# li199603/easy_gaussian_splatting

Hardware: AMD Instinct MI355X
Metric: train iters/sec + forward render fps, 1M Gaussians @ 1080p (higher is better)
Workload: dtype f32

## Files before the change

### easy_gaussian_splatting_amd/csrc/gs_blend.hip

```cpp
#include <algorithm>

#include "gs_common.h"
#include "gs_math.h"

namespace gs {

#ifdef GS_BWD_CHECK
struct BwdCheck {
    float* fwd_T;
    int32_t* fwd_cnt;
    float2* unit_out;
    int2* unit_hdr;
};
static BwdCheck g_bwd_check = {nullptr, nullptr, nullptr, nullptr};
#define GS_IF_CHECK(...) __VA_ARGS__
#else
#define GS_IF_CHECK(...)
#endif

constexpr int kUnit = GS_UNIT;
constexpr int kChunk = 8;
constexpr int kUnitLog = 128;
constexpr int kWalkUnits = GS_WALK_UNITS, kWalkStorage = GS_WALK_STORAGE, kWalkRows = GS_WALK_ROWS,
              kWalkFlags = GS_WALK_FLAGS, kWalkSkip = GS_WALK_SKIP;
constexpr int kScanThreads = 256, kScanPerThread = 32, kScanChunk = kScanThreads * kScanPerThread;

struct BlendFwdArgs {
    const int32_t* tile_order;
    int C, W, H, tw, tiles;
    const float4* rec;
    const float* bg;
    const int32_t *isect_offsets, *flatten_ids, *slots;
    float *out_colors, *out_alphas;
    float4* ckpt;
    int2* qlist;
    int32_t* qcnt;
    uint8_t* qmask;
// ... 153 lines not shown
        if (CKPT) {
            const int4 rc = a.trec[2 * (size_t)t], ru = a.trec[2 * (size_t)t + 1];
            cnt[0] = __builtin_amdgcn_readfirstlane(rc.x); cnt[1] = __builtin_amdgcn_readfirstlane(rc.y);
            cnt[2] = __builtin_amdgcn_readfirstlane(rc.z); cnt[3] = __builtin_amdgcn_readfirstlane(rc.w);
            const int ru4[4] = {ru.x, ru.y, ru.z, ru.w};
#pragma unroll
            for (int k = 0; k < 4; ++k) {
                room[k] = -cnt[k] & (kUnit - 1);
                if (lane == 0 && cnt[k] > 0) uring[4 * k + (((cnt[k] - 1) / kUnit) & 3)] = ru4[k];
            }
        }
    }
    const float qxlo[2] = {(float)x0 + 0.5f, (float)x0 + 8.5f}, qxhi[2] = {(float)x0 + 7.5f, (float)x0 + 15.5f};
    const float qylo[2] = {(float)y0 + 0.5f, (float)y0 + 8.5f}, qyhi[2] = {(float)y0 + 7.5f, (float)y0 + 15.5f};

    auto publish = [&]() {
        if (log_n == 0) return;
        int base = 0;
        if (lane == 0) base = atomicAdd(a.walk + kWalkUnits, log_n);
        base = __builtin_amdgcn_readfirstlane(base);
        __builtin_amdgcn_wave_barrier();
        for (int j = lane; j < log_n; j += 64) {
            const int2 e = ulog[j];
            if (base + j < a.cap_units) a.unit_desc[base + j] = make_int4(4 * t + (e.y & 3), e.y >> 2, e.x, 0);
        }
        __builtin_amdgcn_wave_barrier();
        log_n = 0;
    };

    for (int b = 0; b < nb; ++b) {
        bool qa[4];
#pragma unroll
        for (int k = 0; k < 4; ++k) qa[k] = __builtin_amdgcn_ballot_w64(px_live(T[k])) != 0ull;
        if (!(qa[0] || qa[1] || qa[2] || qa[3])) break;
        if (CKPT && log_n > kUnitLog - 8) publish();
        const int first = lo + b * GS_BUCKET;
        const int m = min(GS_BUCKET, hi - first);
        bool hx[2] = {false, false}, hy[2] = {false, false};
        int my_gid = 0, my_slot = 0;
        if (lane < m) {
            my_gid = a.flatten_ids[first + lane];
            if (CKPT) my_slot = a.slots[first + lane];
            const float4* r = a.rec + 3 * (size_t)my_gid;
            const float4 q0 = r[0], q1 = r[1], q2 = r[2];
            srec[lane * 3] = q0; srec[lane * 3 + 1] = q1; srec[lane * 3 + 2] = q2;
            const float ex = q1.z, ey = q1.w;
#pragma unroll
// ... 32 lines not shown
                    const bool ok = px_live(T[k]) && sigma >= 0.f && alpha >= kAlphaMin;
                    const float am = ok ? alpha : 0.f;
                    if (CKPT) {
                        if (__builtin_amdgcn_ballot_w64(ok) != 0ull) {
                            if (__builtin_expect(room[k] == 0, 0)) {
                                const int pos = cnt[k] + (int)__popcll(cq[k]);
                                if (pool_left == 0) {
                                    int base = 0;
                                    if (lane == 0) base = atomicAdd(range_ctr, kChunk);
                                    base = __builtin_amdgcn_readfirstlane(base);
                                    if (base + kChunk > range_len) {
                                        if (lane == 0) {
                                            atomicOr(a.walk + kWalkFlags, GS_FLAG_UNITS);
                                            if (ROUND != 1 && a.flags) atomicOr(a.flags, (unsigned long long)GS_FLAG_UNITS);
                                        }
                                        base = 0;
                                    }
                                    pool_next = range0 + base; pool_left = kChunk;
                                }
                                const int su = pool_next++;
                                --pool_left;
                                a.ckpt[(size_t)su * 64 + lane] = make_float4(px_live(T[k]) ? T[k] : -1.f, cr[k], cg[k], cb[k]);
                                if constexpr (NC == 4) ckpt_ext[(size_t)su * 64 + lane] = ca[k];
                                if (lane == 0) ulog[log_n] = make_int2(su, (pos / kUnit) * 4 + k);
                                ++log_n;
                                if (lane == 0) uring[4 * k + ((pos / kUnit) & 3)] = su;
                                room[k] = kUnit;
                            }
                            --room[k];
                            cq[k] |= 1ull << j;
                        }
                    }
                    GS_IF_CHECK(const float T_before = T[k];)
                    if constexpr (NC == 4) blend_masked4(am, r, g, bl, q2.w, T[k], cr[k], cg[k], cb[k], ca[k]);
                    else blend_masked(am, r, g, bl, T[k], cr[k], cg[k], cb[k]);
                    GS_IF_CHECK(taken[k] += T[k] < T_before ? 1 : 0;)
                }
            }
        }
        if (CKPT) {
            int mybits = 0;
#pragma unroll
            for (int k = 0; k < 4; ++k) {
                const int n_new = (int)__popcll(cq[k]);
                if ((cq[k] >> lane) & 1) {
                    const int p = cnt[k] + (int)__popcll(cq[k] & lt_mask);
                    const int su = uring[4 * k + ((p / kUnit) & 3)];
// ... 149 lines not shown
    const int32_t tot = row_counts32(a.qmask, i0, n, w);
    int32_t block_tot;
    const int32_t run = block_excl_scan_add<int32_t>(tot, scratch, &block_tot) + a.walk[GS_WALK_WORDS + blockIdx.x];
    int32_t first16 = 0;
#pragma unroll
    for (int j = 0; j < 4; ++j) first16 += (int32_t)((w[j] * 0x01010101u) >> 24);
    if (i0 <= n) a.row_base[i0 >> 4] = run;
    if (i0 + 16 <= n) a.row_base[(i0 >> 4) + 1] = run + first16;
}

struct BlendBwdArgs {
    int C, W, H, tw, tiles;
    const float4* rec;
    const int32_t* walk;
    const int2* qlist;
    const int32_t* qcnt;
    const int4* unit_desc;
    const float4* ckpt;
    const uint8_t* qmask;
    const int32_t* row_base;
    int cap_units;
    const int32_t* cls_hdr;
    const int4* cls_desc;
    int cls_cap;
    const float *out_colors, *out_alphas, *v_colors, *v_alphas;
    float4* rows;
    const int64_t* guard;
    GS_IF_CHECK(BwdCheck chk;)
};

constexpr int kBwdWaves = 4;
constexpr int kPipeLanes = 8;
constexpr int kPerLane = kUnit / kPipeLanes;
static_assert(kPerLane == 4, "bwd_wave is instantiated for 1 .. 4 entries per lane");
constexpr int kUnitsPerWave = 64 / kPipeLanes;
constexpr int kUnitPixels = 64;
constexpr int kBwdSteps = kUnitPixels + kPipeLanes - 1;

__device__ __forceinline__ float dpp_row_shr1(float v) {
    return __builtin_bit_cast(float, __builtin_amdgcn_update_dpp(__builtin_bit_cast(int, v), __builtin_bit_cast(int, v), 0x111, 0xf, 0xf, false));
}


#ifdef GS_BWD_ACC64
typedef double acc_t;
#define GS_ACC_FMA(a, b, c) ((double)(a) * (double)(b) + (c))
#else
typedef float acc_t;
#define GS_ACC_FMA(a, b, c) fmaf((a), (b), (c))
#endif
struct EntryState {
    float mx, my, hA, Bc, hC, op, colr, colg, colb, At, Bt, Ct;
    acc_t s_mx, s_my, s_ax, s_ay, s_A, s_B, s_C, s_vs, s_r, s_g, s_b;
    bool has;
    float col3; acc_t s_3;
};

template <int NC>
__device__ __forceinline__ void bwd_pair(EntryState& e, const float4 d0, const float v3, const float2 d1, float& T, float& P) {
    const float dx = e.mx - d1.x, dy = e.my - d1.y;
// ... 6 lines not shown
    const float Tn = fmaf(-alpha, T, T);
    const bool stop = ok && Tn <= kTMin;
    const bool contrib = ok && !stop;
    float cv = e.colr * d0.x + e.colg * d0.y + e.colb * d0.z;
    if constexpr (NC == 4) cv = fmaf(e.col3, v3, cv);
    const float wm = contrib ? w : 0.f;
    const float Pn = fmaf(wm, cv, P);
    const float ra = fast_rcp(1.f - alpha);
    const float v_alpha = fmaf(T, cv, ra * (d0.w + Pn));
    e.s_r = GS_ACC_FMA(wm, d0.x, e.s_r); e.s_g = GS_ACC_FMA(wm, d0.y, e.s_g); e.s_b = GS_ACC_FMA(wm, d0.z, e.s_b);
    if constexpr (NC == 4) e.s_3 = GS_ACC_FMA(wm, v3, e.s_3);
    const float vs = (contrib && ov <= kAlphaMax) ? -ov * v_alpha : 0.f;
    const float hx = vs * dx, hy = vs * dy;
    e.s_A = GS_ACC_FMA(hx, dx, e.s_A); e.s_B = GS_ACC_FMA(hx, dy, e.s_B); e.s_C = GS_ACC_FMA(hy, dy, e.s_C);
    const float gx = fmaf(e.At, hx, e.Bt * hy), gy = fmaf(e.Bt, hx, e.Ct * hy);
    e.s_mx += (acc_t)gx; e.s_my += (acc_t)gy; e.s_ax += (acc_t)fabsf(gx); e.s_ay += (acc_t)fabsf(gy);
    e.s_vs += (acc_t)vs;
    T = contrib ? Tn : (stop ? -1.f : T);
    P = Pn;
}

template <int E, int NC>
__device__ __forceinline__ void bwd_wave(const BlendBwdArgs& a, const int4 ud, const bool valid, const int unit, float4* sd0, float* sd1,
                                         float2* sck, const int r, const float* __restrict__ ckpt_ext) {
    const int tq = ud.x, su = ud.z;
    const bool first_unit = ud.y == 0;
    const int t = tq >> 2, q = tq & 3;
    const int cam = t / a.tiles, tt = t - cam * a.tiles;
    const int tyi = tt / a.tw, txi = tt - tyi * a.tw;
    const int qx0 = txi * GS_TILE + 8 * (q & 1), qy0 = tyi * GS_TILE + 8 * (q >> 1);
    const float fx0 = (float)qx0 + 0.5f, fy0 = (float)qy0 + 0.5f;
    const float4* ckp = a.ckpt + (size_t)su * 64;

    const int n_sub = valid ? a.qcnt[tq] : 0;
    int2 gs[E];
    {
        const int2* qp2 = a.qlist + (size_t)su * kUnit + E * r;
        if constexpr (E == 4) {
            const int4* qp = reinterpret_cast<const int4*>(qp2);
            const int4 g0 = qp[0], g1 = qp[1];
            gs[0] = make_int2(g0.x, g0.y); gs[1] = make_int2(g0.z, g0.w); gs[2] = make_int2(g1.x, g1.y); gs[3] = make_int2(g1.z, g1.w);
        } else if constexpr (E == 2) {
            const int4 g0 = *reinterpret_cast<const int4*>(qp2);
            gs[0] = make_int2(g0.x, g0.y); gs[1] = make_int2(g0.z, g0.w);
        } else {
#pragma unroll
            for (int i = 0; i < E; ++i) gs[i] = qp2[i];
// ... 8 lines not shown
    for (int i = 0; i < kPix; ++i) {
        const int p = r + kPipeLanes * i;
        const int px = min(qx0 + (p & 7), a.W - 1), py = min(qy0 + (p >> 3), a.H - 1);
        const size_t o = ((size_t)cam * a.H + py) * a.W + px;
        l_vr[i] = a.v_colors[NC * o];
        l_vg[i] = NC > 1 ? a.v_colors[NC * o + 1] : 0.f;
        l_vb[i] = NC > 2 ? a.v_colors[NC * o + 2] : 0.f;
        l_oa[i] = a.out_alphas[o];
        l_cr[i] = a.out_colors[NC * o];
        l_cg[i] = NC > 1 ? a.out_colors[NC * o + 1] : 0.f;
        l_cb[i] = NC > 2 ? a.out_colors[NC * o + 2] : 0.f;
        l_va[i] = vap[o];
        l_ck[i] = ckp[p];
        if constexpr (NC == 4) { l_v3[i] = a.v_colors[NC * o + 3]; l_c3[i] = a.out_colors[NC * o + 3]; l_k3[i] = ckpt_ext[(size_t)su * 64 + p]; }
    }
    const int n_in = min(kPipeLanes * E, n_sub - ud.y * kUnit);
    float4 rq[E][3];
#pragma unroll
    for (int i = 0; i < E; ++i) {
        const bool has = E * r + i < n_in;
        const float4* rp = a.rec + 3 * (size_t)(has ? gs[i].x : 0);
        rq[i][0] = rp[0]; rq[i][1] = rp[1]; rq[i][2] = rp[2];
    }
#pragma unroll
    for (int i = 0; i < kPix; ++i) {
        const int p = r + kPipeLanes * i;
        const bool inside = valid && (qx0 + (p & 7)) < a.W && (qy0 + (p >> 3)) < a.H;
        const float vr = l_vr[i], vg = l_vg[i], vb = l_vb[i];
        const float Tf = 1.f - l_oa[i];
        const float va = a.v_alphas ? l_va[i] : 0.f;
        float Ev = Tf * va - (l_cr[i] * vr + l_cg[i] * vg + l_cb[i] * vb);
        const float4 ck = first_unit ? make_float4(1.f, 0.f, 0.f, 0.f) : l_ck[i];
        float Pk = ck.y * vr + ck.z * vg + ck.w * vb;
        if constexpr (NC == 4) {
            const float v3 = l_v3[i];
            Ev = Tf * va - fmaf(l_c3[i], v3, l_cr[i] * vr + l_cg[i] * vg + l_cb[i] * vb);
            Pk = fmaf(first_unit ? 0.f : l_k3[i], v3, Pk);
            sd1[p] = inside ? v3 : 0.f;
        }
        sd0[p] = inside ? make_float4(vr, vg, vb, Ev) : make_float4(0.f, 0.f, 0.f, 0.f);
        sck[p] = inside ? make_float2(ck.x, Pk) : make_float2(-1.f, 0.f);
    }

    EntryState e[E];
    int slot[E];
#pragma unroll
    for (int i = 0; i < E; ++i) {
        const int en = E * r + i;
        e[i].has = en < n_in;
        slot[i] = e[i].has ? gs[i].y : 0;
        const float4 z4 = make_float4(0.f, 0.f, 0.f, 0.f);
        const float4 q0 = e[i].has ? rq[i][0] : z4, q1 = e[i].has ? rq[i][1] : z4, q2 = e[i].has ? rq[i][2] : z4;
        e[i].mx = q0.x; e[i].my = q0.y; e[i].hA = q0.z; e[i].Bc = q0.w; e[i].hC = q1.x; e[i].op = q1.y;
        e[i].colr = q2.x; e[i].colg = q2.y; e[i].colb = q2.z;
        e[i].col3 = q2.w; e[i].s_3 = (acc_t)0;
        e[i].At = 2.f * kLn2 * q0.z; e[i].Bt = kLn2 * q0.w; e[i].Ct = 2.f * kLn2 * q1.x;
        e[i].s_mx = e[i].s_my = e[i].s_ax = e[i].s_ay = e[i].s_A = e[i].s_B = e[i].s_C = e[i].s_vs = (acc_t)0;
        e[i].s_r = e[i].s_g = e[i].s_b = (acc_t)0;
    }
    __builtin_amdgcn_wave_barrier();

    float T_out = -1.f, P_out = 0.f;
    GS_IF_CHECK(float D_out = -1.f, C_out = 0.f; if (valid && r == 0 && a.chk.unit_hdr) a.chk.unit_hdr[unit] = make_int2(tq, ud.y);)
    for (int s = 0; s < kBwdSteps; ++s) {
        float T = dpp_row_shr1(T_out), P = dpp_row_shr1(P_out);
        const int p = s - r;
        const bool act = (unsigned)p < (unsigned)kUnitPixels;
        const int pc = min(max(p, 0), kUnitPixels - 1);
        const float4 d0 = sd0[pc];
        const float v3 = NC == 4 ? sd1[pc] : 0.f;
        const float2 ck = sck[pc];
        const float2 d1 = make_float2(fx0 + (float)(pc & 7), fy0 + (float)(pc >> 3));
        if (r == 0) { T = ck.x; P = ck.y; }
        T = act ? T : -1.f;
        GS_IF_CHECK(float D = dpp_row_shr1(D_out), Cn = dpp_row_shr1(C_out); if (r == 0) { D = ck.x; Cn = 0.f; } if (!act) { D = -1.f; Cn = 0.f; })
#pragma unroll
        for (int i = 0; i < E; ++i) {
            GS_IF_CHECK(const float T_before = T;)
            bwd_pair<NC>(e[i], d0, v3, d1, T, P);
            GS_IF_CHECK(if (T > 0.f && T < T_before) { D = T; Cn += 1.f; })
        }
        GS_IF_CHECK(D_out = D; C_out = Cn;
                    if (valid && act && r == kPipeLanes - 1 && a.chk.unit_out) a.chk.unit_out[(size_t)unit * 64 + p] = make_float2(D, Cn);)
        T_out = T; P_out = P;
    }

    int row[E];
#pragma unroll
    for (int i = 0; i < E; ++i) {
        int m;
        row[i] = rows_before(a.row_base, a.qmask, slot[i], &m);
        row[i] += __popc((unsigned)m & ((1u << q) - 1u));
    }
#pragma unroll
    for (int i = 0; i < E; ++i) {
        if (e[i].has) {
            float4* rp = a.rows + (GS_ROW_FLOATS / 4) * (size_t)row[i];
            const float v_op = e[i].op > 0.f ? (float)(-e[i].s_vs / (acc_t)e[i].op) : 0.f;
            rp[0] = make_float4((float)e[i].s_mx, (float)e[i].s_my, (float)e[i].s_ax, (float)e[i].s_ay);
            rp[1] = make_float4((float)((acc_t)0.5f * e[i].s_A), (float)e[i].s_B, (float)((acc_t)0.5f * e[i].s_C), v_op);
            rp[2] = make_float4((float)e[i].s_r, (float)e[i].s_g, (float)e[i].s_b, NC == 4 ? (float)e[i].s_3 : 0.f);
        }
    }
}

constexpr int kClsHdrInts = 16, kClsThreads = 1024;
__global__ __launch_bounds__(64) void unit_classes_clear_kernel(int32_t* __restrict__ hdr) {
    if (threadIdx.x < kClsHdrInts) hdr[threadIdx.x] = 0;
}
__global__ __launch_bounds__(kClsThreads) void unit_classes_kernel(const int32_t* __restrict__ walk, const int4* __restrict__ unit_desc,
                                                                   const int32_t* __restrict__ qcnt, int cap_units, int cls_cap,
                                                                   int32_t* __restrict__ hdr, int4* __restrict__ cls, const int64_t* __restrict__ guard) {
    __shared__ int s_cnt[kClsThreads / 64][4], s_base[kClsThreads / 64][4];
    if (guard_tripped(guard)) return;
    const int n_units = min(walk[kWalkUnits], cap_units);
    if ((int)blockIdx.x * kClsThreads >= n_units) return;
    const int u = (int)blockIdx.x * kClsThreads + (int)threadIdx.x, wave = threadIdx.x >> 6, lane = threadIdx.x & 63;
    int c = 0;
    int4 ud = make_int4(0, 0, 0, 0);
    if (u < n_units) {
        ud = unit_desc[u];
        const int n_in = min(kUnit, qcnt[ud.x] - ud.y * kUnit);
        c = min(max((n_in + kPipeLanes - 1) / kPipeLanes, 1), 4);
        ud.w = u;
    }
    unsigned long long m[4];
#pragma unroll
    for (int k = 0; k < 4; ++k) m[k] = __ballot(c == k + 1);
    if (lane < 4) s_cnt[wave][lane] = (int)__popcll(lane == 0 ? m[0] : (lane == 1 ? m[1] : (lane == 2 ? m[2] : m[3])));
    __syncthreads();
    if (threadIdx.x < 4) {
        int tot = 0;
        for (int w = 0; w < kClsThreads / 64; ++w) { s_base[w][threadIdx.x] = tot; tot += s_cnt[w][threadIdx.x]; }
        const int base = tot ? atomicAdd(hdr + 1 + threadIdx.x, tot) : 0;
        for (int w = 0; w < kClsThreads / 64; ++w) s_base[w][threadIdx.x] += base;
    }
    __syncthreads();
    if (c) {
        const unsigned long long mine = c == 1 ? m[0] : (c == 2 ? m[1] : (c == 3 ? m[2] : m[3]));
        const int i = s_base[wave][c - 1] + (int)__popcll(mine & ((1ull << lane) - 1ull));
        if (i < (c == 4 ? cap_units : cls_cap)) cls[(c == 4 ? 0 : cap_units + (3 - c) * cls_cap) + i] = ud;
    }
}

template <int NC>
__device__ __forceinline__ void blend_bwd_body(const BlendBwdArgs& a, const float* __restrict__ ckpt_ext) {
    __shared__ float4 sd0_all[kBwdWaves][kUnitsPerWave][64];
    __shared__ float2 sck_all[kBwdWaves][kUnitsPerWave][64];
    const int wave = threadIdx.x >> 6, lane = threadIdx.x & 63;
    const int pipe = lane / kPipeLanes, r = lane & (kPipeLanes - 1);
    if (guard_tripped(a.guard)) return;
    constexpr int kPerBlock = kBwdWaves * kUnitsPerWave;
    int cls = 4, blk = (int)blockIdx.x, n_units, first = 0;
    if (a.cls_hdr == nullptr) {
        n_units = min(a.walk[kWalkUnits], a.cap_units);
    } else {
        const int b4 = (a.cap_units + kPerBlock - 1) / kPerBlock, bt = (a.cls_cap + kPerBlock - 1) / kPerBlock;
        if (blk >= b4) {
            const int k = (blk - b4) / bt;
            cls = 3 - k; blk -= b4 + k * bt; first = a.cap_units + k * a.cls_cap;
        }
        n_units = min(a.cls_hdr[cls], cls == 4 ? a.cap_units : a.cls_cap);
    }
    const int in_class = (blk * kBwdWaves + wave) * kUnitsPerWave + pipe;
    if ((blk * kBwdWaves + wave) * kUnitsPerWave >= n_units) return;
    GS_CLOCK_PROBE_SCOPE(2);
    const bool valid = in_class < n_units;
    float4* sd0 = sd0_all[wave][pipe];
    float2* sck = sck_all[wave][pipe];
    float* sd1 = nullptr;
    if constexpr (NC == 4) {
        __shared__ float sd1_all[kBwdWaves][kUnitsPerWave][64];
        sd1 = sd1_all[wave][pipe];
    }

    int4 ud = make_int4(0, 0, 0, 0);
    if (valid) ud = a.cls_hdr ? a.cls_desc[first + in_class] : a.unit_desc[in_class];
    const int unit = a.cls_hdr ? ud.w : in_class;
    if (cls == 4) bwd_wave<4, NC>(a, ud, valid, unit, sd0, sd1, sck, r, ckpt_ext);
    else if (cls == 3) bwd_wave<3, NC>(a, ud, valid, unit, sd0, sd1, sck, r, ckpt_ext);
    else if (cls == 2) bwd_wave<2, NC>(a, ud, valid, unit, sd0, sd1, sck, r, ckpt_ext);
    else bwd_wave<1, NC>(a, ud, valid, unit, sd0, sd1, sck, r, ckpt_ext);
}

__global__ __launch_bounds__(kBwdWaves * 64) void blend_bwd_kernel(const BlendBwdArgs a) {
    blend_bwd_body<3>(a, nullptr);
}
template <int NC>
__global__ __launch_bounds__(kBwdWaves * 64) void chan_bwd_kernel(const BlendBwdArgs a, const float* ckpt_ext) {
    blend_bwd_body<NC>(a, ckpt_ext);
}

}

using namespace gs;

#ifdef GS_BWD_CHECK
extern "C" int gs_debug_bwd_check_set(float* fwd_T, int32_t* fwd_cnt, float* unit_out, int32_t* unit_hdr) {
    g_bwd_check.fwd_T = fwd_T; g_bwd_check.fwd_cnt = fwd_cnt;
    g_bwd_check.unit_out = reinterpret_cast<float2*>(unit_out); g_bwd_check.unit_hdr = reinterpret_cast<int2*>(unit_hdr);
    return GS_OK;
}
#endif

#ifdef GS_CLOCK_PROBE
extern "C" int gs_debug_clock_probe(int64_t* out4, int reset) {
    unsigned long long h[4] = {0, 0, 0, 0};
    if (out4) { GS_HIP_CHECK(hipMemcpyFromSymbol(h, HIP_SYMBOL(gs_clk_acc), sizeof(h))); for (int i = 0; i < 4; ++i) out4[i] = (int64_t)h[i]; }
    if (reset) { unsigned long long z[4] = {0, 0, 0, 0}; GS_HIP_CHECK(hipMemcpyToSymbol(HIP_SYMBOL(gs_clk_acc), z, sizeof(z))); }
    return GS_OK;
}
#endif

extern "C" size_t gs_walk_state_ints(int64_t n_isects) {
    if (n_isects < 0) return 0;
    return (size_t)GS_WALK_WORDS + (size_t)(n_isects / kScanChunk + 1);
}

template <int NC>
static int blend_fwd_launch(void* stream, int C, int width, int height, const float* rec,
                            const float* backgrounds, const int32_t* isect_offsets, const int32_t* tile_order,
                            const int32_t* flatten_ids, const int32_t* slots, int64_t n_isects, float* render_colors,
                            float* render_alphas, float* ckpt, int32_t* qlist, int32_t* qcnt, uint8_t* qmask,
// ... 110 lines not shown
                            const int32_t* qlist, const int32_t* qcnt, const int32_t* unit_desc, int64_t cap_units,
                            const float* ckpt, const uint8_t* qmask, const int32_t* row_base, const int32_t* walk_state,
                            const float* render_colors, const float* render_alphas, const float* v_render_colors,
                            const float* v_render_alphas, float* rows, int32_t* unit_classes, const float* ckpt_ext) {
    GS_REQUIRE(C >= 1 && width > 0 && height > 0 && cap_units >= 0 && cap_units < (1ll << 26), "C>=1, positive image size, 0 <= cap_units < 2^26");
    if (cap_units == 0) return GS_OK;
    GS_REQUIRE(rec && qlist && qcnt && unit_desc && ckpt && qmask && row_base && walk_state, "null list pointer");
    GS_REQUIRE(render_colors && render_alphas && v_render_colors && rows, "null image pointer");
    GS_REQUIRE(NC != 4 || ckpt_ext, "channels = 4: ckpt_ext (gs_blend_fwd_ch's fourth-channel checkpoints) is required");
    BlendBwdArgs a;
    a.C = C; a.W = width; a.H = height;
    a.tw = (width + GS_TILE - 1) / GS_TILE;
    a.tiles = a.tw * ((height + GS_TILE - 1) / GS_TILE);
    a.rec = reinterpret_cast<const float4*>(rec);
    a.qlist = reinterpret_cast<const int2*>(qlist); a.qcnt = qcnt; a.walk = walk_state;
    a.unit_desc = reinterpret_cast<const int4*>(unit_desc); a.cap_units = (int)cap_units;
    a.ckpt = reinterpret_cast<const float4*>(ckpt); a.qmask = qmask; a.row_base = row_base;
    a.out_colors = render_colors;
    a.out_alphas = render_alphas; a.v_colors = v_render_colors; a.v_alphas = v_render_alphas;
    a.rows = reinterpret_cast<float4*>(rows);
    a.guard = current_guard().info;
    GS_IF_CHECK(a.chk = g_bwd_check;)
    unsigned grid = (unsigned)((cap_units + kUnitsPerWave * kBwdWaves - 1) / (kUnitsPerWave * kBwdWaves));
    a.cls_hdr = nullptr; a.cls_desc = nullptr; a.cls_cap = 0;
    if (unit_classes) {
        GS_REQUIRE(((uintptr_t)unit_classes & 15) == 0, "unit_classes must be 16-byte aligned");
        a.cls_hdr = unit_classes; a.cls_desc = reinterpret_cast<const int4*>(unit_classes + kClsHdrInts);
        a.cls_cap = (int)cls_region(C, width, height);
        hipLaunchKernelGGL(unit_classes_clear_kernel, dim3(1), dim3(64), 0, (hipStream_t)stream, unit_classes);
        hipLaunchKernelGGL(unit_classes_kernel, dim3((unsigned)((cap_units + kClsThreads - 1) / kClsThreads)), dim3(kClsThreads), 0, (hipStream_t)stream,
                           walk_state, a.unit_desc, qcnt, (int)cap_units, a.cls_cap, unit_classes, reinterpret_cast<int4*>(unit_classes + kClsHdrInts),
                           a.guard);
        GS_LAUNCH_CHECK("unit_classes_kernel");
        grid += 3u * (unsigned)(a.cls_cap / (kUnitsPerWave * kBwdWaves));
    }
    if constexpr (NC == 3) hipLaunchKernelGGL(blend_bwd_kernel, dim3(grid), dim3(kBwdWaves * 64), 0, (hipStream_t)stream, a);
    else hipLaunchKernelGGL((chan_bwd_kernel<NC>), dim3(grid), dim3(kBwdWaves * 64), 0, (hipStream_t)stream, a, ckpt_ext);
    GS_LAUNCH_CHECK("blend_bwd_kernel");
    return GS_OK;
}

extern "C" int gs_blend_bwd(void* stream, int C, int width, int height, const float* rec,
                            const int32_t* qlist, const int32_t* qcnt, const int32_t* unit_desc, int64_t cap_units,
                            const float* ckpt, const uint8_t* qmask, const int32_t* row_base, const int32_t* walk_state,
                            const float* render_colors, const float* render_alphas, const float* v_render_colors,
                            const float* v_render_alphas, float* rows, int32_t* unit_classes) {
    return blend_bwd_launch<3>(stream, C, width, height, rec, qlist, qcnt, unit_desc, cap_units, ckpt, qmask, row_base, walk_state,
                               render_colors, render_alphas, v_render_colors, v_render_alphas, rows, unit_classes, nullptr);
}

extern "C" int gs_blend_bwd_ch(void* stream, int C, int width, int height, int channels, const float* rec,
                               const int32_t* qlist, const int32_t* qcnt, const int32_t* unit_desc, int64_t cap_units,
                               const float* ckpt, const uint8_t* qmask, const int32_t* row_base, const int32_t* walk_state,
                               const float* render_colors, const float* render_alphas, const float* v_render_colors,
                               const float* v_render_alphas, float* rows, int32_t* unit_classes, const float* ckpt_ext) {
    GS_REQUIRE(channels >= 1 && channels <= 4, "channels must be 1, 2, 3 or 4");
#define GS_BWD_CH(NC) blend_bwd_launch<NC>(stream, C, width, height, rec, qlist, qcnt, unit_desc, cap_units, ckpt, qmask, row_base, \
// ... 11 lines not shown
```

### easy_gaussian_splatting_amd/rendering.py

```python
from __future__ import annotations

import ctypes as _ct
import math
import os
import threading
import time
import weakref
from typing import Dict, Optional, Tuple

import torch
from torch import Tensor

from . import _native as nat
from . import workspace as WS

_TILE = nat.GS_TILE
_BWD_CLASSES = os.environ.get("GS_BWD_CLASSES", "1") != "0"


def _ptr(t: Optional[Tensor]) -> Optional[int]:
    return None if t is None else t.data_ptr()


def _stream(device: torch.device) -> int:
# ... 397 lines not shown
    coarse_cap, shift, flags = lay.key[5:8]
    if flags & WS.F_TWO_LEVEL:
        check(L.gs_bins_lists(st, C, N, tw, th, shift, bbox, P(WS.BIN), lay.extent(WS.BIN), P(WS.COARSE_KEYS), coarse_cap, P(WS.CUM_TILES),
                              P(WS.ISECT_OFFSETS), P(WS.ISECT_IDS), P(WS.FLATTEN_IDS), P(WS.SLOTS), P(WS.INFO)), "gs_bins_lists")
    else:
        check(L.gs_bin_emit_sort(st, C, N, tw, th, bbox, depths, P(WS.BIN), lay.extent(WS.BIN), P(WS.ISECT_OFFSETS), n_isects, max_tile_count,
                                 P(WS.KEYS_TMP), P(WS.SLOT_GID), P(WS.CUM_TILES), P(WS.ISECT_IDS), P(WS.FLATTEN_IDS), P(WS.SLOTS)), "gs_bin_emit_sort")


def _ckpt_ext(lease, ch: int):
    return lease.ckpt_ext() if (ch == 4 and lease.layout.key[7] & WS.F_TRAIN) else None


def stage_blend_fwd(L, st, lease, C, W, H, ch, backgrounds, n_isects, colors, alphas, check=nat.check):
    P, lay = lease.ptr, lease.layout
    common = (P(WS.REC), backgrounds, P(WS.ISECT_OFFSETS), P(WS.TILE_ORDER), P(WS.FLATTEN_IDS), P(WS.SLOTS), n_isects, colors, alphas, P(WS.CKPT),
              P(WS.QLIST), P(WS.QCNT), P(WS.QMASK), P(WS.UNIT_DESC), lay.cap_units, P(WS.ROW_BASE), lay.cap_rows, P(WS.WALK_STATE))
    if ch == 3:
        check(L.gs_blend_fwd(st, C, W, H, *common), "gs_blend_fwd")
    else:
        check(L.gs_blend_fwd_ch(st, C, W, H, ch, *common, _ckpt_ext(lease, ch)), "gs_blend_fwd_ch")


def stage_blend_bwd(L, st, lease, C, W, H, ch, colors, alphas, v_colors, v_alphas, unit_classes, check=nat.check):
    P = lease.ptr
    common = (P(WS.REC), P(WS.QLIST), P(WS.QCNT), P(WS.UNIT_DESC), lease.layout.cap_units, P(WS.CKPT), P(WS.QMASK), P(WS.ROW_BASE),
              P(WS.WALK_STATE), colors, alphas, v_colors, v_alphas, P(WS.ROWS), unit_classes)
    if ch == 3:
        check(L.gs_blend_bwd(st, C, W, H, *common), "gs_blend_bwd")
    else:
        check(L.gs_blend_bwd_ch(st, C, W, H, ch, *common, _ckpt_ext(lease, ch)), "gs_blend_bwd_ch")


def _forward_stages(means, quats, scales, opacities, colors, colors_rest, viewmats, Ks, backgrounds, cfg, need_grad):
    L = nat.lib()
    dev = means.device
    C, N = viewmats.shape[0], means.shape[0]
    W, H = cfg["width"], cfg["height"]
    sh_degree = cfg["sh_degree"]
    tw, th = math.ceil(W / _TILE), math.ceil(H / _TILE)
    tiles = tw * th
    st = _stream(dev)
    f32 = dict(dtype=torch.float32, device=dev)
    i32 = dict(dtype=torch.int32, device=dev)

    if sh_degree is None:
        deg, K = -1, 0
        per_cam = 1 if colors.dim() == 3 else 0
    else:
# ... 302 lines not shown
    with _state_lock:
        old = _hints.get(s["hint_key"])
        if old is not None:
            old["cap_units"] = max(storage + (storage >> 2) + 512, int(old.get("cap_units", 0) * 0.995))
            old["cap_rows"] = max(rows + (rows >> 2) + 4096, int(old.get("cap_rows", 0) * 0.995))
    return rows


class _Rasterize(torch.autograd.Function):

    @staticmethod
    def forward(ctx, means, quats, scales, opacities, colors, colors_rest, viewmats, Ks, backgrounds, cfg, holder, campos=None):
        ctx.camera_grads = bool(cfg.get("camera_grads")) and ctx.needs_input_grad[6]
        need_grad = bool(cfg.get("grad_enabled", True)) and (any(ctx.needs_input_grad[:6]) or ctx.camera_grads)
        ctx.set_materialize_grads(False)
        render_colors, render_alphas, meta, state = _forward_stages(
            means, quats, scales, opacities, colors, colors_rest, viewmats, Ks, backgrounds, cfg, need_grad)
        holder.meta = meta
        if holder.debug is not None and need_grad:
            lease, tiles = state["lease"], meta["tile_width"] * meta["tile_height"]
            wstate = lease.view(WS.WALK_STATE, 8).clone()
            holder.debug.update(unit_counter=wstate[WS.WALK_UNITS:WS.WALK_UNITS + 1], walk_state=wstate,
                                qcnt=lease.view(WS.QCNT, state["C"] * tiles * 4).clone(), unit_entries=nat.GS_UNIT)
            if state["n_isects"] is not None:
                holder.debug["walked_isects"] = lease.view(WS.QMASK, max(state["n_isects"], 1))[: state["n_isects"]].count_nonzero()
        holder.lease_ref = state.pop("lease_ref")
        out_colors = render_colors
        if cfg.get("expected_depth"):
            out_colors = torch.empty_like(render_colors)
            _stage("gs_expected_depth_fwd", means.device, lambda: nat.check(nat.lib().gs_expected_depth_fwd(
                _stream(means.device), render_alphas.numel(), state["ch"], _ptr(render_colors), _ptr(render_alphas), _ptr(out_colors)),
                "gs_expected_depth_fwd"))
        holder.out_ptrs = (out_colors.data_ptr(), render_alphas.data_ptr())
        ctx.cfg, ctx.holder, ctx.state = cfg, holder, state
        ctx.split = colors_rest is not None
        if need_grad:
            extra = (colors_rest,) if ctx.split else ()
            ctx.save_for_backward(means, quats, scales, colors, viewmats, Ks, render_colors, render_alphas, opacities, *extra)
        return out_colors, render_alphas

    @staticmethod
    def backward(ctx, v_render_colors, v_render_alphas):
        L = nat.lib()
        means, quats, scales, colors, viewmats, Ks, render_colors, render_alphas, opacities = ctx.saved_tensors[:9]
        colors_rest = ctx.saved_tensors[9] if ctx.split else None
        s, cfg, holder = ctx.state, ctx.cfg, ctx.holder
        dev = means.device
        st = _stream(dev)
        C, N, K = s["C"], s["N"], s["K"]
        W, H = cfg["width"], cfg["height"]
        f32 = dict(dtype=torch.float32, device=dev)
        v_rc = torch.zeros_like(render_colors) if v_render_colors is None else v_render_colors.contiguous()
        v_ra = None if v_render_alphas is None else v_render_alphas.contiguous()
        lease, factorised = s["lease"], s["factorised"]
        if s.get("pending") is not None:
            if s["pending"].resolve():
                raise RuntimeError("rasterization(_size_check='deferred'): the forward of this call outgrew its list capacities and was "
                                   "repaired only now -- the loss and the upstream gradient of this backward were computed from unwritten "
                                   "memory.  Re-run the step (the capacities have been raised), or use the default immediate size check.")
            s["n_isects"], s["n_buckets"] = s["late"]["n_isects"], s["late"]["n_buckets"]
        P = lease.ptr
        n_rows = _settle_walk(s, cfg, render_colors, render_alphas)
        ucls = torch.empty((int(L.gs_unit_classes_ints(lease.layout.cap_units, C, W, H)),), dtype=torch.int32, device=dev) if _BWD_CLASSES else None
        ch, dc, dmode = s["ch"], s["dc"], s["dmode"]
        if cfg.get("expected_depth"):
            v_out, v_ra_in = v_rc, v_ra
            v_rc, v_ra = torch.empty_like(render_colors), torch.empty_like(render_alphas)
            _stage("gs_expected_depth_bwd", dev, lambda: nat.check(L.gs_expected_depth_bwd(
                st, render_alphas.numel(), ch, _ptr(render_colors), _ptr(render_alphas), _ptr(v_out), _ptr(v_ra_in), _ptr(v_rc), _ptr(v_ra)),
                "gs_expected_depth_bwd"))
        _stage("gs_blend_bwd", dev, lambda: stage_blend_bwd(L, st, lease, C, W, H, ch, _ptr(render_colors), _ptr(render_alphas), _ptr(v_rc), _ptr(v_ra),
                                                            _ptr(ucls)))
        go = holder.grad_out or {}
        for k_, shp in (("means", (N, 3)), ("quats", (N, 4)), ("scales", (N, 3)), ("opacities", (N,)), ("grad_norm", (N,)), ("count", (N,))):
            if k_ in go and not (go[k_].shape == shp and go[k_].is_contiguous() and go[k_].dtype == torch.float32 and go[k_].device == dev):
                raise ValueError(f"_grad_out['{k_}'] must be a contiguous float32 tensor of shape {shp} on {dev}")
        if ("grad_norm" in go) != ("count" in go) or ("count" in go and not (factorised and C == 1)):
            raise ValueError("_grad_out['grad_norm'] / ['count'] come together, with _sh_grads='colors_pre' and a single camera")
        v_means = go["means"] if "means" in go else torch.empty((N, 3), **f32)
        v_quats = go["quats"] if "quats" in go else torch.empty((N, 4), **f32)
        v_scales = go["scales"] if "scales" in go else torch.empty((N, 3), **f32)
        v_opac = go["opacities"] if "opacities" in go else torch.empty((N,), **f32)
        v_colors = None if (factorised or dmode == "only") else torch.empty(colors.shape, **f32)
        v_pc, pc_cam = (v_colors, s["per_cam"]) if dc == 3 else (torch.empty((C, N, 3), **f32), 1)
        v_rest = torch.empty(colors_rest.shape, **f32) if (ctx.split and not factorised and dmode != "only") else None
        v_pre = row_sums = None
        if factorised:
            row_sums = torch.empty((C * N, 12), **f32)
            pay = holder.view_payload
            if pay is not None:
                if not (C == 1 and pay.dim() == 1 and pay.numel() >= 4 * N + 16 and pay.is_contiguous() and pay.dtype == torch.float32 and pay.device == dev):
                    raise ValueError(f"_view_payload must be a contiguous 1-D float32 tensor of >= 4 N + 16 elements on {dev} (single camera)")
                v_pre, rad_out, cam_out = pay[:3 * N].view(1, N, 3), pay[3 * N:4 * N], pay[4 * N:4 * N + 16]
            else:
                v_pre, rad_out, cam_out = torch.empty((C, N, 3), **f32), None, None
# ... 250 lines not shown
```

Measured before the change: 732.3.

## Compact live pixels per backward unit and sort units by entry and live-pixel class

The forward pass now records, for each checkpoint unit, how many pixels are still live and packs that count into the unit descriptor. The backward kernel compacts only the live pixels into shared memory, storing their pixel coordinates, and shortens its pipelined step loop to the longest live count among the pipes of the wave. The unit classification becomes a two-kernel counting sort over 32 keys, combining entry count and live-pixel bucket. Units of similar length then share a wave and the per-class grid regions are replaced by one compact grid. This adds a shared-memory pixel index, extra ballots, and one more pre-pass kernel.

```diff
diff --git a/easy_gaussian_splatting_amd/csrc/gs_blend.hip b/easy_gaussian_splatting_amd/csrc/gs_blend.hip
--- a/easy_gaussian_splatting_amd/csrc/gs_blend.hip
+++ b/easy_gaussian_splatting_amd/csrc/gs_blend.hip
@@ -11,8 +11,9 @@
     int32_t* fwd_cnt;
     float2* unit_out;
     int2* unit_hdr;
+    int all_pixels;
 };
-static BwdCheck g_bwd_check = {nullptr, nullptr, nullptr, nullptr};
+static BwdCheck g_bwd_check = {nullptr, nullptr, nullptr, nullptr, 0};
 #define GS_IF_CHECK(...) __VA_ARGS__
 #else
 #define GS_IF_CHECK(...)
@@ -212,7 +213,7 @@
         __builtin_amdgcn_wave_barrier();
         for (int j = lane; j < log_n; j += 64) {
             const int2 e = ulog[j];
-            if (base + j < a.cap_units) a.unit_desc[base + j] = make_int4(4 * t + (e.y & 3), e.y >> 2, e.x, 0);
+            if (base + j < a.cap_units) a.unit_desc[base + j] = make_int4(4 * t + (e.y & 3), e.y >> 2, e.x & ((1 << 26) - 1), (int)((unsigned)e.x >> 26) + 1);
         }
         __builtin_amdgcn_wave_barrier();
         log_n = 0;
@@ -291,7 +292,8 @@
                                 --pool_left;
                                 a.ckpt[(size_t)su * 64 + lane] = make_float4(px_live(T[k]) ? T[k] : -1.f, cr[k], cg[k], cb[k]);
                                 if constexpr (NC == 4) ckpt_ext[(size_t)su * 64 + lane] = ca[k];
-                                if (lane == 0) ulog[log_n] = make_int2(su, (pos / kUnit) * 4 + k);
+                                const int n_live = (int)__popcll(__builtin_amdgcn_ballot_w64(px_live(T[k])));
+                                if (lane == 0) ulog[log_n] = make_int2((int)((unsigned)su | ((unsigned)(n_live - 1) << 26)), (pos / kUnit) * 4 + k);
                                 ++log_n;
                                 if (lane == 0) uring[4 * k + ((pos / kUnit) & 3)] = su;
                                 room[k] = kUnit;
@@ -487,7 +489,6 @@
     int cap_units;
     const int32_t* cls_hdr;
     const int4* cls_desc;
-    int cls_cap;
     const float *out_colors, *out_alphas, *v_colors, *v_alphas;
     float4* rows;
     const int64_t* guard;
@@ -500,7 +501,6 @@
 static_assert(kPerLane == 4, "bwd_wave is instantiated for 1 .. 4 entries per lane");
 constexpr int kUnitsPerWave = 64 / kPipeLanes;
 constexpr int kUnitPixels = 64;
-constexpr int kBwdSteps = kUnitPixels + kPipeLanes - 1;
 
 __device__ __forceinline__ float dpp_row_shr1(float v) {
     return __builtin_bit_cast(float, __builtin_amdgcn_update_dpp(__builtin_bit_cast(int, v), __builtin_bit_cast(int, v), 0x111, 0xf, 0xf, false));
@@ -553,7 +553,7 @@
 
 template <int E, int NC>
 __device__ __forceinline__ void bwd_wave(const BlendBwdArgs& a, const int4 ud, const bool valid, const int unit, float4* sd0, float* sd1,
-                                         float2* sck, const int r, const float* __restrict__ ckpt_ext) {
+                                         float2* sck, uint16_t* spix, const int r, const float* __restrict__ ckpt_ext) {
     const int tq = ud.x, su = ud.z;
     const bool first_unit = ud.y == 0;
     const int t = tq >> 2, q = tq & 3;
@@ -608,10 +608,17 @@
         const float4* rp = a.rec + 3 * (size_t)(has ? gs[i].x : 0);
         rq[i][0] = rp[0]; rq[i][1] = rp[1]; rq[i][2] = rp[2];
     }
+    int n_live = 0;
+    const int pipe_shift = (int)(threadIdx.x & 63) & ~(kPipeLanes - 1);
 #pragma unroll
     for (int i = 0; i < kPix; ++i) {
         const int p = r + kPipeLanes * i;
         const bool inside = valid && (qx0 + (p & 7)) < a.W && (qy0 + (p >> 3)) < a.H;
+        bool live = inside && (first_unit || l_ck[i].x > 0.f);
+        GS_IF_CHECK(live = live || a.chk.all_pixels != 0;)
+        const unsigned mine = (unsigned)(__builtin_amdgcn_ballot_w64(live) >> pipe_shift) & ((1u << kPipeLanes) - 1u);
+        const int place = n_live + __popc(mine & ((1u << r) - 1u));
+        n_live += __popc(mine);
         const float vr = l_vr[i], vg = l_vg[i], vb = l_vb[i];
         const float Tf = 1.f - l_oa[i];
         const float va = a.v_alphas ? l_va[i] : 0.f;
@@ -622,11 +629,24 @@
             const float v3 = l_v3[i];
             Ev = Tf * va - fmaf(l_c3[i], v3, l_cr[i] * vr + l_cg[i] * vg + l_cb[i] * vb);
             Pk = fmaf(first_unit ? 0.f : l_k3[i], v3, Pk);
-            sd1[p] = inside ? v3 : 0.f;
-        }
-        sd0[p] = inside ? make_float4(vr, vg, vb, Ev) : make_float4(0.f, 0.f, 0.f, 0.f);
-        sck[p] = inside ? make_float2(ck.x, Pk) : make_float2(-1.f, 0.f);
-    }
+            if (live) sd1[place] = inside ? v3 : 0.f;
+        }
+        if (live) {
+            sd0[place] = inside ? make_float4(vr, vg, vb, Ev) : make_float4(0.f, 0.f, 0.f, 0.f);
+            sck[place] = inside ? make_float2(ck.x, Pk) : make_float2(-1.f, 0.f);
+            spix[place] = (uint16_t)((p & 7) | ((p >> 3) << 8));
+        }
+        GS_IF_CHECK(if (inside && !live && a.chk.unit_out) a.chk.unit_out[(size_t)unit * 64 + p] = make_float2(-1.f, 0.f);)
+    }
+    if (n_live == 0 && r == 0) {
+        sd0[0] = make_float4(0.f, 0.f, 0.f, 0.f); sck[0] = make_float2(-1.f, 0.f); spix[0] = 0;
+        if constexpr (NC == 4) sd1[0] = 0.f;
+    }
+    int n_steps = 0;
+#pragma unroll
+    for (int k = 0; k < kUnitsPerWave; ++k) n_steps = max(n_steps, __builtin_amdgcn_readlane(n_live, kPipeLanes * k));
+    n_steps += kPipeLanes - 1;
+    const int last = max(n_live - 1, 0);
 
     EntryState e[E];
     int slot[E];
@@ -648,15 +668,16 @@
 
     float T_out = -1.f, P_out = 0.f;
     GS_IF_CHECK(float D_out = -1.f, C_out = 0.f; if (valid && r == 0 && a.chk.unit_hdr) a.chk.unit_hdr[unit] = make_int2(tq, ud.y);)
-    for (int s = 0; s < kBwdSteps; ++s) {
+    for (int s = 0; s < n_steps; ++s) {
         float T = dpp_row_shr1(T_out), P = dpp_row_shr1(P_out);
         const int p = s - r;
-        const bool act = (unsigned)p < (unsigned)kUnitPixels;
-        const int pc = min(max(p, 0), kUnitPixels - 1);
+        const bool act = (unsigned)p < (unsigned)n_live;
+        const int pc = min(max(p, 0), last);
         const float4 d0 = sd0[pc];
         const float v3 = NC == 4 ? sd1[pc] : 0.f;
         const float2 ck = sck[pc];
-        const float2 d1 = make_float2(fx0 + (float)(pc & 7), fy0 + (float)(pc >> 3));
+        const unsigned pix = spix[pc];
+        const float2 d1 = make_float2(fx0 + (float)(pix & 0xffu), fy0 + (float)(pix >> 8));
         if (r == 0) { T = ck.x; P = ck.y; }
         T = act ? T : -1.f;
         GS_IF_CHECK(float D = dpp_row_shr1(D_out), Cn = dpp_row_shr1(C_out); if (r == 0) { D = ck.x; Cn = 0.f; } if (!act) { D = -1.f; Cn = 0.f; })
@@ -667,7 +688,7 @@
             GS_IF_CHECK(if (T > 0.f && T < T_before) { D = T; Cn += 1.f; })
         }
         GS_IF_CHECK(D_out = D; C_out = Cn;
-                    if (valid && act && r == kPipeLanes - 1 && a.chk.unit_out) a.chk.unit_out[(size_t)unit * 64 + p] = make_float2(D, Cn);)
+                    if (valid && act && r == kPipeLanes - 1 && a.chk.unit_out) a.chk.unit_out[(size_t)unit * 64 + (pix & 7u) + 8u * (pix >> 8)] = make_float2(D, Cn);)
         T_out = T; P_out = P;
     }
 
@@ -690,42 +711,85 @@
     }
 }
 
-constexpr int kClsHdrInts = 16, kClsThreads = 1024;
-__global__ __launch_bounds__(64) void unit_classes_clear_kernel(int32_t* __restrict__ hdr) {
-    if (threadIdx.x < kClsHdrInts) hdr[threadIdx.x] = 0;
-}
-__global__ __launch_bounds__(kClsThreads) void unit_classes_kernel(const int32_t* __restrict__ walk, const int4* __restrict__ unit_desc,
-                                                                   const int32_t* __restrict__ qcnt, int cap_units, int cls_cap,
-                                                                   int32_t* __restrict__ hdr, int4* __restrict__ cls, const int64_t* __restrict__ guard) {
-    __shared__ int s_cnt[kClsThreads / 64][4], s_base[kClsThreads / 64][4];
+constexpr int kClsHdrInts = 16, kClsThreads = 1024, kClsKeys = 32;
+__device__ __forceinline__ int unit_class_key(const int4 ud, const int32_t* __restrict__ qcnt) {
+    const int n_in = min(kUnit, qcnt[ud.x] - ud.y * kUnit);
+    const int e = min(max((n_in + kPipeLanes - 1) / kPipeLanes, 1), 4);
+    const int lc = min(max((ud.w + 7) >> 3, 1), 8);
+    return (e - 1) * 8 + (lc - 1);
+}
+__global__ __launch_bounds__(kClsThreads) void unit_classes_count_kernel(const int32_t* __restrict__ walk, const int4* __restrict__ unit_desc,
+                                                                         const int32_t* __restrict__ qcnt, int cap_units, int32_t* __restrict__ table,
+                                                                         const int64_t* __restrict__ guard) {
+    __shared__ int s_cnt[kClsKeys];
     if (guard_tripped(guard)) return;
     const int n_units = min(walk[kWalkUnits], cap_units);
     if ((int)blockIdx.x * kClsThreads >= n_units) return;
-    const int u = (int)blockIdx.x * kClsThreads + (int)threadIdx.x, wave = threadIdx.x >> 6, lane = threadIdx.x & 63;
-    int c = 0;
+    if (threadIdx.x < kClsKeys) s_cnt[threadIdx.x] = 0;
+    __syncthreads();
+    const int u = (int)blockIdx.x * kClsThreads + (int)threadIdx.x;
+    if (u < n_units) atomicAdd(&s_cnt[unit_class_key(unit_desc[u], qcnt)], 1);
+    __syncthreads();
+    if (threadIdx.x < kClsKeys) table[(size_t)blockIdx.x * kClsKeys + threadIdx.x] = s_cnt[threadIdx.x];
+}
+__global__ __launch_bounds__(kClsThreads) void unit_classes_place_kernel(const int32_t* __restrict__ walk, const int4* __restrict__ unit_desc,
+                                                                         const int32_t* __restrict__ qcnt, int cap_units,
+                                                                         const int32_t* __restrict__ table, int4* __restrict__ cls,
+                                                                         const int64_t* __restrict__ guard) {
+    constexpr int kWavesHere = kClsThreads / 64;
+    __shared__ int s_tot[kClsThreads / kClsKeys][kClsKeys], s_bef[kClsThreads / kClsKeys][kClsKeys];
+    __shared__ int s_wcnt[kWavesHere][kClsKeys];
+    if (guard_tripped(guard)) return;
+    const int n_units = min(walk[kWalkUnits], cap_units);
+    if ((int)blockIdx.x * kClsThreads >= n_units) return;
+    const int n_rows = (n_units + kClsThreads - 1) / kClsThreads;
+    const int wave = threadIdx.x >> 6, lane = threadIdx.x & 63;
+    {
+        const int k = threadIdx.x & (kClsKeys - 1), j = threadIdx.x / kClsKeys;
+        int tot = 0, bef = 0;
+        for (int row = j; row < n_rows; row += kClsThreads / kClsKeys) {
+            const int c = table[(size_t)row * kClsKeys + k];
+            tot += c;
+            bef += row < (int)blockIdx.x ? c : 0;
+        }
+        s_tot[j][k] = tot; s_bef[j][k] = bef;
+    }
+    for (int i = threadIdx.x; i < kWavesHere * kClsKeys; i += kClsThreads) s_wcnt[i / kClsKeys][i % kClsKeys] = 0;
+    __syncthreads();
+    const int u = (int)blockIdx.x * kClsThreads + (int)threadIdx.x;
+    const bool has = u < n_units;
     int4 ud = make_int4(0, 0, 0, 0);
-    if (u < n_units) {
-        ud = unit_desc[u];
-        const int n_in = min(kUnit, qcnt[ud.x] - ud.y * kUnit);
-        c = min(max((n_in + kPipeLanes - 1) / kPipeLanes, 1), 4);
-        ud.w = u;
-    }
-    unsigned long long m[4];
-#pragma unroll
-    for (int k = 0; k < 4; ++k) m[k] = __ballot(c == k + 1);
-    if (lane < 4) s_cnt[wave][lane] = (int)__popcll(lane == 0 ? m[0] : (lane == 1 ? m[1] : (lane == 2 ? m[2] : m[3])));
+    int key = 0;
+    if (has) { ud = unit_desc[u]; key = unit_class_key(ud, qcnt); }
+    unsigned long long same = __ballot(has);
+#pragma unroll
+    for (int b = 0; b < 5; ++b) {
+        const unsigned long long m = __ballot((key >> b) & 1);
+        same &= ((key >> b) & 1) ? m : ~m;
+    }
+    const int rank = (int)__popcll(same & ((1ull << lane) - 1ull));
+    if (has && rank == 0) s_wcnt[wave][key] = (int)__popcll(same);
     __syncthreads();
-    if (threadIdx.x < 4) {
-        int tot = 0;
-        for (int w = 0; w < kClsThreads / 64; ++w) { s_base[w][threadIdx.x] = tot; tot += s_cnt[w][threadIdx.x]; }
-        const int base = tot ? atomicAdd(hdr + 1 + threadIdx.x, tot) : 0;
-        for (int w = 0; w < kClsThreads / 64; ++w) s_base[w][threadIdx.x] += base;
+    if (threadIdx.x < kClsKeys) {
+        const int k = threadIdx.x;
+        int tot = 0, run = 0;
+#pragma unroll
+        for (int j = 0; j < kClsThreads / kClsKeys; ++j) { tot += s_tot[j][k]; run += s_bef[j][k]; }
+        int suffix = tot;
+#pragma unroll
+        for (int d = 1; d < kClsKeys; d <<= 1) {
+            const int up = __shfl_down(suffix, d, 64);
+            suffix += k + d < kClsKeys ? up : 0;
+        }
+        run += suffix - tot;
+#pragma unroll
+        for (int w = 0; w < kWavesHere; ++w) { const int c = s_wcnt[w][k]; s_wcnt[w][k] = run; run += c; }
     }
     __syncthreads();
-    if (c) {
-        const unsigned long long mine = c == 1 ? m[0] : (c == 2 ? m[1] : (c == 3 ? m[2] : m[3]));
-        const int i = s_base[wave][c - 1] + (int)__popcll(mine & ((1ull << lane) - 1ull));
-        if (i < (c == 4 ? cap_units : cls_cap)) cls[(c == 4 ? 0 : cap_units + (3 - c) * cls_cap) + i] = ud;
+    if (has) {
+        const int i = s_wcnt[wave][key] + rank;
+        ud.w = u | (((key >> 3) + 1) << 26);
+        if (i < cap_units) cls[i] = ud;
     }
 }
 
@@ -736,24 +800,15 @@
     const int wave = threadIdx.x >> 6, lane = threadIdx.x & 63;
     const int pipe = lane / kPipeLanes, r = lane & (kPipeLanes - 1);
     if (guard_tripped(a.guard)) return;
-    constexpr int kPerBlock = kBwdWaves * kUnitsPerWave;
-    int cls = 4, blk = (int)blockIdx.x, n_units, first = 0;
-    if (a.cls_hdr == nullptr) {
-        n_units = min(a.walk[kWalkUnits], a.cap_units);
-    } else {
-        const int b4 = (a.cap_units + kPerBlock - 1) / kPerBlock, bt = (a.cls_cap + kPerBlock - 1) / kPerBlock;
-        if (blk >= b4) {
-            const int k = (blk - b4) / bt;
-            cls = 3 - k; blk -= b4 + k * bt; first = a.cap_units + k * a.cls_cap;
-        }
-        n_units = min(a.cls_hdr[cls], cls == 4 ? a.cap_units : a.cls_cap);
-    }
-    const int in_class = (blk * kBwdWaves + wave) * kUnitsPerWave + pipe;
-    if ((blk * kBwdWaves + wave) * kUnitsPerWave >= n_units) return;
+    const int n_units = min(a.walk[kWalkUnits], a.cap_units);
+    const int first = ((int)blockIdx.x * kBwdWaves + wave) * kUnitsPerWave, in_class = first + pipe;
+    if (first >= n_units) return;
     GS_CLOCK_PROBE_SCOPE(2);
     const bool valid = in_class < n_units;
+    __shared__ uint16_t spix_all[kBwdWaves][kUnitsPerWave][64];
     float4* sd0 = sd0_all[wave][pipe];
     float2* sck = sck_all[wave][pipe];
+    uint16_t* spix = spix_all[wave][pipe];
     float* sd1 = nullptr;
     if constexpr (NC == 4) {
         __shared__ float sd1_all[kBwdWaves][kUnitsPerWave][64];
@@ -761,12 +816,13 @@
     }
 
     int4 ud = make_int4(0, 0, 0, 0);
-    if (valid) ud = a.cls_hdr ? a.cls_desc[first + in_class] : a.unit_desc[in_class];
-    const int unit = a.cls_hdr ? ud.w : in_class;
-    if (cls == 4) bwd_wave<4, NC>(a, ud, valid, unit, sd0, sd1, sck, r, ckpt_ext);
-    else if (cls == 3) bwd_wave<3, NC>(a, ud, valid, unit, sd0, sd1, sck, r, ckpt_ext);
-    else if (cls == 2) bwd_wave<2, NC>(a, ud, valid, unit, sd0, sd1, sck, r, ckpt_ext);
-    else bwd_wave<1, NC>(a, ud, valid, unit, sd0, sd1, sck, r, ckpt_ext);
+    if (valid) ud = a.cls_hdr ? a.cls_desc[in_class] : a.unit_desc[in_class];
+    const int unit = a.cls_hdr ? (ud.w & ((1 << 26) - 1)) : in_class;
+    const int cls = a.cls_hdr ? min(max(__builtin_amdgcn_readfirstlane(ud.w) >> 26, 1), 4) : 4;
+    if (cls == 4) bwd_wave<4, NC>(a, ud, valid, unit, sd0, sd1, sck, spix, r, ckpt_ext);
+    else if (cls == 3) bwd_wave<3, NC>(a, ud, valid, unit, sd0, sd1, sck, spix, r, ckpt_ext);
+    else if (cls == 2) bwd_wave<2, NC>(a, ud, valid, unit, sd0, sd1, sck, spix, r, ckpt_ext);
+    else bwd_wave<1, NC>(a, ud, valid, unit, sd0, sd1, sck, spix, r, ckpt_ext);
 }
 
 __global__ __launch_bounds__(kBwdWaves * 64) void blend_bwd_kernel(const BlendBwdArgs a) {
@@ -785,6 +841,10 @@
 extern "C" int gs_debug_bwd_check_set(float* fwd_T, int32_t* fwd_cnt, float* unit_out, int32_t* unit_hdr) {
     g_bwd_check.fwd_T = fwd_T; g_bwd_check.fwd_cnt = fwd_cnt;
     g_bwd_check.unit_out = reinterpret_cast<float2*>(unit_out); g_bwd_check.unit_hdr = reinterpret_cast<int2*>(unit_hdr);
+    return GS_OK;
+}
+extern "C" int gs_debug_bwd_all_pixels(int on) {
+    g_bwd_check.all_pixels = on ? 1 : 0;
     return GS_OK;
 }
 #endif
@@ -941,17 +1001,18 @@
     a.guard = current_guard().info;
     GS_IF_CHECK(a.chk = g_bwd_check;)
     unsigned grid = (unsigned)((cap_units + kUnitsPerWave * kBwdWaves - 1) / (kUnitsPerWave * kBwdWaves));
-    a.cls_hdr = nullptr; a.cls_desc = nullptr; a.cls_cap = 0;
-    if (unit_classes) {
-        GS_REQUIRE(((uintptr_t)unit_classes & 15) == 0, "unit_classes must be 16-byte aligned");
-        a.cls_hdr = unit_classes; a.cls_desc = reinterpret_cast<const int4*>(unit_classes + kClsHdrInts);
-        a.cls_cap = (int)cls_region(C, width, height);
-        hipLaunchKernelGGL(unit_classes_clear_kernel, dim3(1), dim3(64), 0, (hipStream_t)stream, unit_classes);
-        hipLaunchKernelGGL(unit_classes_kernel, dim3((unsigned)((cap_units + kClsThreads - 1) / kClsThreads)), dim3(kClsThreads), 0, (hipStream_t)stream,
-                           walk_state, a.unit_desc, qcnt, (int)cap_units, a.cls_cap, unit_classes, reinterpret_cast<int4*>(unit_classes + kClsHdrInts),
-                           a.guard);
-        GS_LAUNCH_CHECK("unit_classes_kernel");
-        grid += 3u * (unsigned)(a.cls_cap / (kUnitsPerWave * kBwdWaves));
+    a.cls_hdr = nullptr; a.cls_desc = nullptr;
+    const int64_t cls_blocks = (cap_units + kClsThreads - 1) / kClsThreads;
+    GS_REQUIRE(((uintptr_t)unit_classes & 15) == 0, "unit_classes must be 16-byte aligned");
+    if (unit_classes && cls_blocks * kClsKeys <= 48 * (int64_t)C * a.tiles) {
+        int4* cls = reinterpret_cast<int4*>(unit_classes + kClsHdrInts);
+        int32_t* table = unit_classes + kClsHdrInts + 4 * cap_units;
+        a.cls_hdr = unit_classes; a.cls_desc = cls;
+        hipLaunchKernelGGL(unit_classes_count_kernel, dim3((unsigned)cls_blocks), dim3(kClsThreads), 0, (hipStream_t)stream, walk_state, a.unit_desc,
+                           qcnt, (int)cap_units, table, a.guard);
+        hipLaunchKernelGGL(unit_classes_place_kernel, dim3((unsigned)cls_blocks), dim3(kClsThreads), 0, (hipStream_t)stream, walk_state, a.unit_desc,
+                           qcnt, (int)cap_units, (const int32_t*)table, cls, a.guard);
+        GS_LAUNCH_CHECK("unit_classes_place_kernel");
     }
     if constexpr (NC == 3) hipLaunchKernelGGL(blend_bwd_kernel, dim3(grid), dim3(kBwdWaves * 64), 0, (hipStream_t)stream, a);
     else hipLaunchKernelGGL((chan_bwd_kernel<NC>), dim3(grid), dim3(kBwdWaves * 64), 0, (hipStream_t)stream, a, ckpt_ext);
diff --git a/easy_gaussian_splatting_amd/rendering.py b/easy_gaussian_splatting_amd/rendering.py
--- a/easy_gaussian_splatting_amd/rendering.py
+++ b/easy_gaussian_splatting_amd/rendering.py
@@ -443,9 +443,9 @@
         check(L.gs_blend_fwd_ch(st, C, W, H, ch, *common, _ckpt_ext(lease, ch)), "gs_blend_fwd_ch")
 
 
-def stage_blend_bwd(L, st, lease, C, W, H, ch, colors, alphas, v_colors, v_alphas, unit_classes, check=nat.check):
+def stage_blend_bwd(L, st, lease, C, W, H, ch, colors, alphas, v_colors, v_alphas, unit_classes, check=nat.check, cap_units=None):
     P = lease.ptr
-    common = (P(WS.REC), P(WS.QLIST), P(WS.QCNT), P(WS.UNIT_DESC), lease.layout.cap_units, P(WS.CKPT), P(WS.QMASK), P(WS.ROW_BASE),
+    common = (P(WS.REC), P(WS.QLIST), P(WS.QCNT), P(WS.UNIT_DESC), lease.layout.cap_units if cap_units is None else cap_units, P(WS.CKPT), P(WS.QMASK), P(WS.ROW_BASE),
               P(WS.WALK_STATE), colors, alphas, v_colors, v_alphas, P(WS.ROWS), unit_classes)
     if ch == 3:
         check(L.gs_blend_bwd(st, C, W, H, *common), "gs_blend_bwd")
@@ -794,6 +794,11 @@
             wstate = lease.view(WS.WALK_STATE, 8).clone()
             holder.debug.update(unit_counter=wstate[WS.WALK_UNITS:WS.WALK_UNITS + 1], walk_state=wstate,
                                 qcnt=lease.view(WS.QCNT, state["C"] * tiles * 4).clone(), unit_entries=nat.GS_UNIT)
+            if holder.debug.get("walk"):
+                n_units = min(int(wstate[WS.WALK_UNITS]), lease.layout.cap_units)
+                desc = lease.view(WS.UNIT_DESC, lease.layout.cap_units * 4).view(-1, 4)[:n_units].clone()
+                holder.debug.update(unit_desc=desc, cap_units=lease.layout.cap_units,
+                                    ckpt=lease.view(WS.CKPT, lease.layout.cap_units * 256).view(-1, 64, 4)[desc[:, 2].long()])
             if state["n_isects"] is not None:
                 holder.debug["walked_isects"] = lease.view(WS.QMASK, max(state["n_isects"], 1))[: state["n_isects"]].count_nonzero()
         holder.lease_ref = state.pop("lease_ref")
@@ -833,7 +838,8 @@
             s["n_isects"], s["n_buckets"] = s["late"]["n_isects"], s["late"]["n_buckets"]
         P = lease.ptr
         n_rows = _settle_walk(s, cfg, render_colors, render_alphas)
-        ucls = torch.empty((int(L.gs_unit_classes_ints(lease.layout.cap_units, C, W, H)),), dtype=torch.int32, device=dev) if _BWD_CLASSES else None
+        cap_bwd = min(lease.layout.cap_units, int((holder.debug or {}).get("bwd_cap_units") or lease.layout.cap_units))
+        ucls = torch.empty((int(L.gs_unit_classes_ints(cap_bwd, C, W, H)),), dtype=torch.int32, device=dev) if _BWD_CLASSES else None
         ch, dc, dmode = s["ch"], s["dc"], s["dmode"]
         if cfg.get("expected_depth"):
             v_out, v_ra_in = v_rc, v_ra
@@ -842,7 +848,7 @@
                 st, render_alphas.numel(), ch, _ptr(render_colors), _ptr(render_alphas), _ptr(v_out), _ptr(v_ra_in), _ptr(v_rc), _ptr(v_ra)),
                 "gs_expected_depth_bwd"))
         _stage("gs_blend_bwd", dev, lambda: stage_blend_bwd(L, st, lease, C, W, H, ch, _ptr(render_colors), _ptr(render_alphas), _ptr(v_rc), _ptr(v_ra),
-                                                            _ptr(ucls)))
+                                                            _ptr(ucls), cap_units=cap_bwd))
         go = holder.grad_out or {}
         for k_, shp in (("means", (N, 3)), ("quats", (N, 4)), ("scales", (N, 3)), ("opacities", (N,)), ("grad_norm", (N,)), ("count", (N,))):
             if k_ in go and not (go[k_].shape == shp and go[k_].is_contiguous() and go[k_].dtype == torch.float32 and go[k_].device == dev):
```

After: 729.3. Within noise of the previous version (-0.4%).
